# cvxopt/smcp

Hardware: AMD Instinct MI355X
Metric: Newton KKT solves/sec (higher is better)
Workload: dtype f64; 1 GPU; synth50k nested block-arrow SDP n=50000, 8073 cliques, m=100; kktsolver=chol, n=50000, cliques=8073, m=100, blkval_doubles=2493568, update_doubles=10689536, parallelism=single

## Files before the change

smcp_amd/csrc/capi.hip:

```cpp
#include <hip/hip_runtime.h>
#include <memory>
#include <unordered_map>

#include <algorithm>
#include <chrono>
#include <cstdio>
#include <cstring>
#include <map>
#include <new>
#include <atomic>
#include <thread>
#include <type_traits>
#include <vector>

#include "../../include/smcp_amd.h"
#include "context.hpp"
#include "switches.hpp"
#include "front_generic.hip"
#include "front_mfma.hip"
#include "front_large.hip"
#include "front_inv.hip"
#include "front_n16.hip"
#include "front_fam.hip"
#include "front_fam2.hip"
// ... 21 lines not shown
  KID_chol_level = 0, KID_llt_level, KID_pinv_level, KID_gather_level, KID_completion_all,
  KID_hess_up_level, KID_hess_down_level, KID_hess_down_inv_all, KID_hess_up_inv_level, KID_scale_an,
  KID_factor_yaa, KID_trsm_fwd_level, KID_trsm_bwd_level, KID_amap, KID_aadj, KID_scatter_constraints,
  KID_dense_potrf, KID_dense_potrs, KID_vec_axpby, KID_axpby, KID_reduce_cliques, KID_reduce_final,
  KID_hess_up_mfma, KID_hess_down_mfma, KID_chol_mfma, KID_pinv_mfma, KID_prep_lk,
  KID_hess_up_mfma_hbm, KID_hess_down_mfma_hbm, KID_chol_mfma_hbm, KID_pinv_mfma_hbm,
  KID_gram_partial, KID_gram_reduce, KID_hess_up_pad,
  KID_lf_assemble, KID_lf_clear_upd, KID_lf_up1, KID_lf_up2, KID_lf_up3, KID_lf_down1, KID_lf_down2, KID_lf_down3,
  KID_lf_pinv1, KID_lf_pinv2, KID_lf_diag, KID_lf_chol_panel, KID_lf_chol_trail, KID_lf_pack_upd,
  KID_lf_prep_s, KID_lf_prep_row, KID_lf_prep_k, KID_factor_yaa_lds,
  KID_factor_inverse, KID_hess_down_inv_mfma, KID_hess_down_inv_mfma_hbm, KID_hess_up_inv_mfma, KID_hess_up_inv_mfma_hbm,
  KID_completion_mfma, KID_completion_mfma_hbm, KID_lf_copy_an, KID_lf_ri_an, KID_lf_dinv1, KID_lf_dinv2,
  KID_lf_uinv1, KID_lf_uinv2, KID_lf_completion, KID_hess_up_n16, KID_llt_mfma, KID_llt_mfma_hbm, KID_lf_llt,
  KID_hess_up_fam, KID_qr_rmul, KID_qr_dots, KID_qr_comb, KID_qr_small, KID_fam2_prep, KID_mid_chol, KID_lf_diag_inv, KID_lfsp_up, KID_lfsp_prep, KID_leaf_gram, KID_leaf_tables, KID_fam_sparse, KID_gram_diag128, KID_lf_assemble_lds, KID_fam_terms, KID_famt_prep, KID_lf_assemble_lds_dyn, KID_lf_zsp, KID_fam_terms_grp, KID_lf_assemble_fz, KID_factor_inverse_lds, KID_chol_flow,
  KID_mrc_diag, KID_mrc_rank, KID_mrc_reduce, KID_mrc_factor, KID_cut_signs, KID_cut_weights,
  KID_edm_rank, KID_edm_reduce, KID_edm_factor, KID_edm_dense,
  KID_COUNT
};
const char* const KID_NAMES[KID_COUNT] = {
  "k_chol_level", "k_llt_level", "k_pinv_level", "k_gather_level", "k_completion_all",
  "k_hess_up_level", "k_hess_down_level", "k_hess_down_inv_all", "k_hess_up_inv_level", "k_scale_an",
  "k_factor_yaa", "k_trsm_fwd_level", "k_trsm_bwd_level", "k_amap", "k_aadj", "k_scatter_constraints",
  "k_dense_potrf", "k_dense_potrs", "k_vec_axpby", "k_axpby", "k_reduce_cliques", "k_reduce_final",
  "k_hess_up_mfma<true>", "k_hess_down_mfma<true>", "k_chol_mfma<true>", "k_pinv_mfma<true>", "k_prep_lk",
  "k_hess_up_mfma<false>", "k_hess_down_mfma<false>", "k_chol_mfma<false>", "k_pinv_mfma<false>",
  "k_gram_partial", "k_gram_reduce", "k_hess_up_pad",
  "k_lf_assemble", "k_lf_clear_upd", "k_lf_up1", "k_lf_up2", "k_lf_up3", "k_lf_down1", "k_lf_down2", "k_lf_down3",
  "k_lf_pinv1", "k_lf_pinv2", "k_lf_diag", "k_lf_chol_panel", "k_lf_chol_trail", "k_lf_pack_upd",
  "k_lf_prep_s", "k_lf_prep_row", "k_lf_prep_k", "k_factor_yaa_lds",
  "k_factor_inverse", "k_hess_down_inv_mfma<true>", "k_hess_down_inv_mfma<false>", "k_hess_up_inv_mfma<true>",
  "k_hess_up_inv_mfma<false>", "k_completion_mfma<true>", "k_completion_mfma<false>", "k_lf_copy_an", "k_lf_ri_an",
  "k_lf_dinv1", "k_lf_dinv2", "k_lf_uinv1", "k_lf_uinv2", "k_lf_completion", "k_hess_up_n16",
  "k_llt_mfma<true>", "k_llt_mfma<false>", "k_lf_llt", "k_hess_up_fam",
  "k_stack_trsm", "k_stack_dots", "k_stack_comb", "k_qr_small", "k_fam2_prep", "k_mid_chol", "k_lf_diag_inv", "k_lfsp_up", "k_lfsp_prep", "k_leaf_pairs", "k_leaf_tables", "k_fam_sparse", "k_gram_diag128", "k_lf_assemble_lds", "k_fam_terms", "k_famt_prep", "k_lf_assemble_lds_dyn", "k_lf_zsp", "k_fam_terms_grp", "k_lf_assemble_fz", "k_factor_inverse_lds", "k_chol_flow",
  "k_mrc_diag", "k_mrc_rank", "k_mrc_reduce", "k_mrc_factor", "k_cut_signs", "k_cut_weights",
  "k_edm_rank", "k_edm_reduce", "k_edm_factor", "k_edm_dense"};

inline void note_launch(csp_ctx* c, int kid) {
  const hipError_t e = hipGetLastError();
  if (e != hipSuccess && !c->launch_err) {
    c->launch_err = (int)e;
    fprintf(stderr, "smcp_amd: launch of %s failed: %s\n", (kid >= 0 && kid < KID_COUNT) ? KID_NAMES[kid] : "?", hipGetErrorString(e));
  }
}
inline hipError_t end_call(csp_ctx* c) {
  hipError_t e = hipGetLastError();
  if (e == hipSuccess && c->launch_err) e = c->launch_err > 0 ? (hipError_t)c->launch_err : hipErrorLaunchFailure;
  c->launch_err = 0;
  return e;
}

// ... 888 lines not shown
  DeviceCtx& D = c->D;
  const int cnn = std::max(1, a.famcnn), csa = 16 * std::max(1, (a.famcna + 15) / 16);
  const int64_t lim = (160 * 1024 - 1024) / 8;
  const int64_t fixed = fam2_layout<NAT>(cnn, csa).oTab;
  if (fixed + fam2_tail_doubles(4, 9) + 64 > lim) return false;
  static bool attr = false;
  if (!attr) {
    if (hipFuncSetAttribute((const void*)k_fam_sparse<NAT, KSN, true>, hipFuncAttributeMaxDynamicSharedMemorySize, 160 * 1024 - 1024) != hipSuccess) return false;
    if (hipFuncSetAttribute((const void*)k_fam_sparse<NAT, KSN, false>, hipFuncAttributeMaxDynamicSharedMemorySize, 160 * 1024 - 1024) != hipSuccess) return false;
    if (hipFuncSetAttribute((const void*)k_fam2_prep, hipFuncAttributeMaxDynamicSharedMemorySize, 160 * 1024 - 1024) != hipSuccess) return false;
    attr = true;
  }
  const int64_t need = (int64_t)cnt * fam2_const_doubles(cnn, csa);
  if (D.famc_len < need) {
    if (D.famc) { if (hipFree(D.famc) != hipSuccess) return false; D.bytes -= D.famc_len * 8; }
    D.famc = nullptr; D.famc_len = 0;
    if (dev_alloc(&D.famc, need, D.bytes)) return false;
    D.famc_len = need;
  }
  const int ncu = D.ncu;
  int g = 1;
  int64_t best = -1;
  for (int gc = 1; gc <= std::min(nrhs, 32); ++gc) {
    const int64_t rounds = ((int64_t)cnt * gc + ncu - 1) / ncu;
    const int64_t passes = (nrhs + gc - 1) / gc;
    const int64_t cost = rounds * ((passes + 1) / 2 + 4);
    if (best < 0 || cost < best) { best = cost; g = gc; }
  }
  const int passes = (nrhs + g - 1) / g;
  const double avg = 9.0 * (double)D.cnnz / ((double)c->S.nsn * (double)std::max<int64_t>(1, D.m));
  int tabpasses = std::min(passes, 113);
  while (tabpasses > 4 && fixed + fam2_tail_doubles(tabpasses, 9) + (int64_t)(1.5 * avg * tabpasses) + 8 > lim) tabpasses = (tabpasses + 1) / 2;
  const int64_t left = lim - fixed - fam2_tail_doubles(tabpasses, 9) - 4;
  const int ecap = (int)std::max<int64_t>(0, (left * 2) / 3 - 2);
  if (9 * D.kc_maxlist > ecap) return false;
  launch_lds(c, KID_fam2_prep, k_fam2_prep, dim3(cnt), dim3(512), (size_t)8 * fam2_child_layout(cnn, csa).cstride * sizeof(double), st,
             a, D.famc, cnn, csa);
  MfmaArgs a2 = a;
  { static int stag = -1; if (stag < 0) { const char* e = sw_str("SMCP_FAM2_STAG"); stag = e ? atoi(e) : 0; } a2.dn = stag; }
  if (D.lg_request) {
    launch_lds(c, KID_fam_sparse, k_fam_sparse<NAT, KSN, false>, dim3(cnt, g), dim3(512), (size_t)lim * 8, st, a2, U, ldu,
               (const double*)D.famc, cnn, csa, (const int32_t*)D.kc_ij, tabpasses, ecap);
    D.lg_nochild = true;
  } else {
    launch_lds(c, KID_fam_sparse, k_fam_sparse<NAT, KSN, true>, dim3(cnt, g), dim3(512), (size_t)lim * 8, st, a2, U, ldu,
               (const double*)D.famc, cnn, csa, (const int32_t*)D.kc_ij, tabpasses, ecap);
  }
  return true;
}
inline bool famt_disabled() {
// ... 10 lines not shown
  const int64_t lim = (160 * 1024 - 1024) / 8;
  const int64_t fixed = famt_layout<NAT>(8 * cnn).total + 8 * famt_desc_doubles() + famt_grp_misc_doubles();
  const int64_t left = lim - fixed - 4;
  if (left <= 0 || famt_prep_doubles<NAT>(cnn) > lim) return -1;
  return (int)std::max<int64_t>(0, (left * 2) / 3 - 2);
}
inline bool famt_grp_fits(int nat, int cnn) {
  int ecap = -1;
  switch (nat) {
    case 1: ecap = famt_grp_ecap<1>(cnn); break;
    case 2: ecap = famt_grp_ecap<2>(cnn); break;
    case 3: ecap = famt_grp_ecap<3>(cnn); break;
    case 4: ecap = famt_grp_ecap<4>(cnn); break;
  }
  return ecap >= FAMT_GMAX * (FAMT_TCAP / 2);
}
template <int NAT>
bool launch_famt(csp_ctx* c, const MfmaArgs& a, int cnt, int nrhs, double* U, int64_t ldu, hipStream_t st) {
  DeviceCtx& D = c->D;
  if (a.famt_ngrp > 0) {
    const int cnn = std::max(1, a.famcnn);
    const FamtL L = famt_layout<NAT>(8 * cnn);
    const int ecap = famt_grp_ecap<NAT>(cnn);
    static bool attrg = false;
    bool ok = !famt_disabled() && D.lg_request && D.fam_maxterms <= FAMT_TCAP / 2 && ecap >= FAMT_GMAX * (FAMT_TCAP / 2);
    if (ok && !attrg) {
      ok = hipFuncSetAttribute((const void*)k_fam_terms_grp<NAT>, hipFuncAttributeMaxDynamicSharedMemorySize, 160 * 1024 - 1024) == hipSuccess &&
           hipFuncSetAttribute((const void*)k_famt_prep<NAT>, hipFuncAttributeMaxDynamicSharedMemorySize, 160 * 1024 - 1024) == hipSuccess;
      attrg = ok;
    }
    const int64_t need = (int64_t)cnt * (FAMT_HDR + L.total);
    if (ok && D.famc_len < need) {
      if (D.famc) { if (hipFree(D.famc) != hipSuccess) ok = false; D.bytes -= D.famc_len * 8; }
      D.famc = nullptr; D.famc_len = 0;
      if (ok && dev_alloc(&D.famc, need, D.bytes)) ok = false;
      if (ok) D.famc_len = need;
    }
    if (!ok) {
      fprintf(stderr, "smcp_amd: grouped family sweep not launchable\n");
      if (!c->launch_err) c->launch_err = -1;
      return true;
    }
    const int gy = std::min(65535, (nrhs + 7) / 8);
    launch_lds(c, KID_famt_prep, k_famt_prep<NAT>, dim3(cnt), dim3(512), (size_t)famt_prep_doubles<NAT>(cnn) * sizeof(double), st, a, D.famc, cnn, (int32_t*)nullptr);
    launch_lds(c, KID_fam_terms_grp, k_fam_terms_grp<NAT>, dim3(a.famt_ngrp, gy), dim3(512), (size_t)(160 * 1024 - 1024), st, a, U, ldu,
               (const double*)D.famc, cnn, (const int32_t*)D.kc_ij, ecap);
    D.lg_nochild = true;
    return true;
  }
  if (famt_disabled() || !D.lg_request) return false;
  const int cnn = std::max(1, a.famcnn);
  const FamtL L = famt_layout<NAT>(8 * cnn);
  const int64_t lim = (160 * 1024 - 1024) / 8;
  const int64_t fixed = L.total + FAMT_NW * famt_desc_doubles() + 6;
  if (!famt_terms_ok(D)) return false;
  if (fixed + 9 * 4 + 64 > lim) return false;
  const int64_t prep_doubles = famt_prep_doubles<NAT>(cnn);
  if (prep_doubles > lim) return false;
  static bool attr = false;
  if (!attr) {
    if (hipFuncSetAttribute((const void*)k_fam_terms<NAT>, hipFuncAttributeMaxDynamicSharedMemorySize, 160 * 1024 - 1024) != hipSuccess) return false;
    if (hipFuncSetAttribute((const void*)k_famt_prep<NAT>, hipFuncAttributeMaxDynamicSharedMemorySize, 160 * 1024 - 1024) != hipSuccess) return false;
    attr = true;
  }
  const int64_t need = (int64_t)cnt * (FAMT_HDR + L.total);
  if (D.famc_len < need) {
    if (D.famc) { if (hipFree(D.famc) != hipSuccess) return false; D.bytes -= D.famc_len * 8; }
    D.famc = nullptr; D.famc_len = 0;
    if (dev_alloc(&D.famc, need, D.bytes)) return false;
    D.famc_len = need;
  }
  const int ncu = D.ncu;
  int g = 1;
  int64_t best = -1;
  for (int gc = 1; gc <= std::min(nrhs, 32); ++gc) {
    const int64_t rounds = ((int64_t)cnt * gc + ncu - 1) / ncu;
    const int64_t passes = (nrhs + gc - 1) / gc;
    const int64_t cost = rounds * (2 * ((passes + FAMT_NW - 1) / FAMT_NW) + 1);
    if (best < 0 || cost < best) { best = cost; g = gc; }
  }
  static int genv = -1;
  if (genv < 0) { const char* e = sw_str("SMCP_FAMT_G"); genv = e ? atoi(e) : 0; }
  if (genv > 0) g = std::min(genv, nrhs);
  const int passes = (nrhs + g - 1) / g;
  const double avg = 9.0 * (double)D.cnnz / ((double)c->S.nsn * (double)std::max<int64_t>(1, D.m));
  int tabpasses = std::min(passes, 113);
  auto tail = [&](int tp) { return (int64_t)2 * ((tp * 9 + 1) & ~1) / 2 + 2; };
  while (tabpasses > 4 && fixed + tail(tabpasses) + (int64_t)(1.5 * 1.5 * avg * tabpasses) + 8 > lim) tabpasses = (tabpasses + 1) / 2;
  const int64_t left = lim - fixed - tail(tabpasses) - 4;
  const int ecap = (int)std::max<int64_t>(0, (left * 2) / 3 - 2);
  if (9 * D.kc_maxlist > ecap) return false;
  if (a.fz_on) {
    static bool attrz = false;
    if (!attrz) attrz = hipFuncSetAttribute((const void*)k_fam_terms<NAT, false>, hipFuncAttributeMaxDynamicSharedMemorySize, 160 * 1024 - 1024) == hipSuccess;
    if (attrz && D.fz_slot) {
      launch_lds(c, KID_famt_prep, k_famt_prep<NAT>, dim3(cnt), dim3(512), (size_t)prep_doubles * sizeof(double), st, a, D.famc, cnn, D.fz_slot);
      launch_lds(c, KID_fam_terms, k_fam_terms<NAT, false>, dim3(cnt, g), dim3(64 * FAMT_NW), (size_t)lim * 8, st, a, U, ldu,
                 (const double*)D.famc, cnn, (const int32_t*)D.kc_ij, tabpasses, ecap);
      D.lg_nochild = true;
      c->fz_live = true; c->fz_nat = NAT; c->fz_cnn = cnn; c->fz_recl = (int64_t)(FAMT_HDR + L.total);
      return true;
    }
  }
  launch_lds(c, KID_famt_prep, k_famt_prep<NAT>, dim3(cnt), dim3(512), (size_t)prep_doubles * sizeof(double), st, a, D.famc, cnn, (int32_t*)nullptr);
  launch_lds(c, KID_fam_terms, k_fam_terms<NAT>, dim3(cnt, g), dim3(64 * FAMT_NW), (size_t)lim * 8, st, a, U, ldu,
             (const double*)D.famc, cnn, (const int32_t*)D.kc_ij, tabpasses, ecap);
  D.lg_nochild = true;
  return true;
}
inline bool fam2_disabled() {
  static int off = -1;
  if (off < 0) { const char* e = sw_str("SMCP_FAM2"); off = (e && e[0] == '0') ? 1 : 0; }
  return off != 0;
}
bool try_fam2(csp_ctx* c, const MfmaArgs& a, int cnt, int nrhs, double* U, int64_t ldu, hipStream_t st) {
  if (fam2_disabled() || !a.kc_ptr || !c->D.kc_ij || a.ymode != 2 || !a.ysc) return false;
  if (c->D.cnnz > (int64_t)4 * c->S.nsn * std::max<int64_t>(1, c->D.m)) return false;
  const int nat = std::max(1, (a.famna + 15) / 16);
  const bool k2 = a.famnn <= 8;
// ... 1263 lines not shown
      c->D.part_valid = false;
      fp_record(c, 2, x, st);
    }
    if (whole) fp_record(c, 1, x, st);
  } else
  for_levels_down(c, [&](const int32_t* lev, int cnt) {
    a.lev = lev;
    launch(c, KID_pinv_level, k_pinv_level, dim3(cnt), dim3(NT), st, a, x);
  });
  HIPCHK(end_call(c));
  return 0;
}

constexpr int SCALING_FAC = 1;
static bool leafgram_ok(csp_ctx* c, int64_t mcols);
static bool scaling_overlap_on() {
  static int on = -1;
  if (on < 0) { const char* e = sw_str("SMCP_SCALING_OVERLAP"); on = (e && e[0] == '0') ? 0 : 1; }
  return on == 1;
}
static int scaling_impl(csp_ctx* c, double* L, double* Y, int flags, hipStream_t st) {
  DeviceCtx& D = c->D;
  const Symbolic& S = c->S;
  const int64_t bl = S.blklen();
  if (c->scal_lstar < 0) {
    int64_t ls = S.nlev;
    while (ls > 0 && c->lvl[(size_t)ls - 1].nI == 0) --ls;
    c->scal_lstar = ls;
    std::vector<int> lev_of((size_t)S.nsn, 0);
    for (int64_t l = 0; l < S.nlev; ++l)
// ... 64 lines not shown
  bool skipped = false;
  auto factor_level = [&](int64_t l, hipStream_t lds_stream, hipStream_t large_stream) {
    for_level_classes(c, l, af, [&](bool lds, MfmaArgs am, int cnt, size_t, int) {
      if (!am.namax) return;
      if (lds) {
        if (l == 0 && skip_children && am.nS > 0) { cnt -= am.nS; skipped = true; if (!cnt) return; }
        const size_t bytes = ((size_t)padld(am.namax) * am.namax + 256 + 8) * sizeof(double);
        launch_lds(c, KID_factor_yaa_lds, k_factor_yaa_lds, dim3(cnt), dim3(fact_threads(am, 256, 2)), bytes, lds_stream, am, (const double*)D.yaa, D.fac);
      } else {
        launch(c, KID_axpby, k_copy_upd_blocks, dim3(cnt, umax1(std::min(64, (am.namax * am.namax + 1023) / 1024))), dim3(256), large_stream,
               am.t, (const double*)D.yaa, D.fac);
        lf_factor_yaa(c, am, cnt, D.fac, large_stream);
      }
    });
  };
  auto pinv_level = [&](int64_t l) {
    for_level_classes(c, l, ap, [&](bool lds, MfmaArgs am, int cnt, size_t bytes, int thr) {
      (void)bytes;
      if (lds) launch_lds(c, KID_pinv_mfma, k_pinv_mfma<true>, dim3(cnt), dim3(fact_threads(am, thr, 1)),
                          (size_t)mfma_lds_doubles_for(WK_PINV, am.nnmax, am.namax) * sizeof(double), st, am, Y);
      else lf_pinv(c, am, cnt, Y, st);
    });
  };
  for (int64_t l = last; l >= lstar; --l) pinv_level(l);
  bool any_large_sep = false;
  for (int64_t l = lstar; l <= last; ++l) if (c->lvl[(size_t)l].nII && c->lvl[(size_t)l].namaxII > 0) any_large_sep = true;
  std::unique_ptr<Fork> f1;
  if (want_fac && any_large_sep && lstar > 0) f1.reset(new Fork(c, st, 0));
  hipStream_t s1 = f1 ? f1->s : st;
  for (int64_t l = lstar - 1; l >= 0; --l) pinv_level(l);
  if (want_fac) {
    for (int64_t l = last; l >= lstar; --l) factor_level(l, s1, s1);
    for (int64_t l = lstar - 1; l >= 0; --l) factor_level(l, st, st);
  }
  if (f1) f1->join();
  D.lk_tag_L = L; D.lk_tag_Y = Y;
  D.yaa_tag = Y;
  D.fac_tag = want_fac ? Y : nullptr;
  D.fac_partial = want_fac && skipped;
  D.faci_tag = nullptr;
  if (want_fac) D.fac_gen++;
  HIPCHK(end_call(c));
  const int rc = fetch_info(c, st);
  if (rc) {
    D.lk_tag_L = D.lk_tag_Y = D.yaa_tag = D.fac_tag = D.faci_tag = nullptr;
    D.part_valid = false;
  }
  return rc;
}
int csp_cholesky_projected_inverse(csp_ctx* c, double* L, double* Y, int with_factors, void* stream) {
  if (int rc = ready(c)) return rc;
  if (!L || !Y || L == Y) return SMCP_EINVAL;
  return scaling_impl(c, L, Y, with_factors ? SCALING_FAC : 0, (hipStream_t)stream);
}

int csp_completion(csp_ctx* c, double* x, void* stream) {
  if (int rc = ready(c)) return rc;
  invalidate_tags(c, x);
  hipStream_t st = (hipStream_t)stream;
  TreeArgs a = tree_args(c);
// ... 654 lines not shown
```

smcp_amd/csrc/context.hpp:

```cpp
#pragma once
#include <hip/hip_runtime.h>

#include <cstdint>
#include <functional>
#include <map>
#include <vector>

#include "symbolic.hpp"

namespace smcp {

struct CliqueDesc {
  int64_t blk;
  int64_t upd;
  int64_t updp;
  int64_t rows;
  int64_t rel;
  int32_t nn, na;
  int32_t parent;
  int32_t chbeg, chend;
  int32_t first;
  int32_t pad;
};

// ... 51 lines not shown
  int32_t* a_c = nullptr;
  int32_t* s_rloc = nullptr;
  int32_t* s_cloc = nullptr;
  int32_t* dlist = nullptr;
  int32_t* slist = nullptr;
  int32_t* kidx = nullptr;
  int64_t md = 0, ns = 0;
  int32_t* kc_ptr = nullptr;
  int32_t* kc_off = nullptr;
  double* kc_val = nullptr;
  int32_t* kc_ij = nullptr;
  int32_t* fz_no = nullptr; int32_t* fz_slot = nullptr; int32_t* fz_ptr = nullptr; int32_t* fz_pk = nullptr; double* fz_s = nullptr;
  int64_t fz_nfam = 0; bool fz_ok = false;
  double* famc = nullptr;
  int64_t famc_len = 0;
  int64_t kc_maxlist = 0;
  int64_t fam_maxterms = 0;
  double fam_meanterms = 0;
  double* vbuf = nullptr;
  double* trsm_x = nullptr; int64_t trsm_x_len = 0;
  int64_t vcols = 0;
  double* hd = nullptr;
  double* hinv = nullptr;
  int64_t hinv_cap = 0, hinv_n = 0;
  const void* hinv_tag = nullptr;
  double* h_pending = nullptr; int64_t h_pending_n = 0, h_pending_ld = 0; hipStream_t h_pending_stream = nullptr;
  double* sw = nullptr;
  double* gpart = nullptr;
  int64_t gpart_len = 0;
  int64_t* gsl_start = nullptr; int32_t* gsl_len = nullptr; int64_t gsl_cap = 0; int gsl_n = 0;
// ... 124 lines not shown
```

smcp_amd/csrc/front_famt.hip:

```cpp
#include <hip/hip_runtime.h>

namespace smcp {

struct FamtL { int oLi, onK, onMK, oRt, oZero, oCN, oCA, oCM, total; };
template <int NAT>
__host__ __device__ inline FamtL famt_layout(int ncol) {
  constexpr int NA = 16 * NAT;
  FamtL L{};
  int o = 0;
  L.oLi = o; o += 256;
  L.onK = o; o += NA * 16;
  L.onMK = o; o += NA * 16;
  L.oRt = o; o += NA * NA;
  L.oZero = o; o += NA;
  L.oCN = o; o += ncol * 16;
  L.oCA = o; o += ncol * NA;
  L.oCM = o; o += ncol * NA;
  L.total = o;
  return L;
}
typedef unsigned int famt_u2 __attribute__((ext_vector_type(2)));
__device__ inline __amdgpu_buffer_rsrc_t famt_rsrc(double* base, int doubles) {
  return __builtin_amdgcn_make_buffer_rsrc(base, 0, doubles * 8, 0x00020000);
}
// ... 117 lines not shown
    hdr[0] = -1; hdr[1] = 1; hdr[2] = 0; hdr[3] = 0; hdr[4] = 0; hdr[5] = 0;
  }
  {
    const int used = __shfl(inc, 7);
    for (int e = tid; e < (ncol - used) * 16; e += 512) T[L.oCN + used * 16 + e] = 0.0;
    for (int e = tid; e < (ncol - used) * NA; e += 512) { T[L.oCA + used * NA + e] = 0.0; T[L.oCM + used * NA + e] = 0.0; }
  }
  if (tid == 0) {
    if (fz_slot && a.fz_no && a.fz_no[k] >= 0) fz_slot[a.fz_no[k]] = (int32_t)blockIdx.x;
    int* const hdr = reinterpret_cast<int*>(out);
    hdr[0] = k; hdr[1] = nn; hdr[2] = na; hdr[3] = nch;
    hdr[4] = (int)(d.blk & 0xffffffffll); hdr[5] = (int)(d.blk >> 32);
    hdr[6] = 0; hdr[7] = 0;
    hdr[8] = (int)(d.updp & 0xffffffffll); hdr[9] = (int)(d.updp >> 32);
  }
}

template <int NTH>
__device__ inline void famt_copy_tables(double* smem, const double* src, int total, int tid) {
  const double2* const s2 = reinterpret_cast<const double2*>(src);
  double2* const d2 = reinterpret_cast<double2*>(smem);
  const int n2 = total >> 1;
  for (int e0 = tid; e0 < n2; e0 += NTH * 8) {
    double2 v[8];
#pragma unroll
    for (int x = 0; x < 8; ++x) v[x] = s2[min(e0 + x * NTH, n2 - 1)];
#pragma unroll
    for (int x = 0; x < 8; ++x) if (e0 + x * NTH < n2) d2[e0 + x * NTH] = v[x];
  }
}
// ... 623 lines not shown
```

smcp_amd/csrc/kkt.hip:

```cpp

namespace {

using namespace smcp;

__global__ void __launch_bounds__(1024) k_amap(int64_t m, const int64_t* cptr, const int64_t* cidx, const double* cwval,
                                               const double* X, int64_t ldx, double* y, int64_t ldy, int64_t pstride) {
  __shared__ double part[16];
  const int lane = threadIdx.x & 63, wave = threadIdx.x >> 6, nthr = blockDim.x;
  const int64_t i = blockIdx.x;
  const int r = blockIdx.y;
  const double* x = X + (int64_t)r * ldx;
  const int64_t c0 = cptr[i], c1 = cptr[i + 1], share = (c1 - c0 + gridDim.z - 1) / gridDim.z;
  const int64_t e0 = c0 + (int64_t)blockIdx.z * share, e1 = e0 + share < c1 ? e0 + share : c1;
  y += (int64_t)blockIdx.z * pstride;
  double acc = 0.0;
  for (int64_t e = e0 + threadIdx.x; e < e1; e += 4 * nthr) {
    double w[4], v[4];
#pragma unroll
    for (int q = 0; q < 4; ++q) {
      const int64_t ee = e + (int64_t)q * nthr;
      w[q] = ee < e1 ? cwval[ee] : 0.0;
      v[q] = ee < e1 ? x[cidx[ee]] : 0.0;
    }
#pragma unroll
// ... 352 lines not shown
  if (m < 1 || !cptr || !cidx || !cval) return SMCP_EINVAL;
  DeviceCtx& D = c->D;
  const Symbolic& S = c->S;
  HIPCHK(hipSetDevice(D.device));
  if (D.h_pending) { if (int rc = flush_pending_potrf(c, D.h_pending_stream, nullptr, false)) return rc; }
  void* old[] = {D.fz_no, D.fz_slot, D.fz_ptr, D.fz_pk, D.fz_s, D.lg_eptr, D.lg_epk, D.lg_ew, D.lg_remap, D.lg_tab, D.cptr, D.cidx, D.cval, D.cwval, D.rpos, D.rptr, D.rcon, D.rval, D.ustack,
                 D.a_r, D.a_c, D.s_rloc, D.s_cloc, D.dlist, D.slist, D.kidx, D.vbuf, D.hd, D.kc_ptr, D.kc_off, D.kc_val, D.kc_ij, D.scm_owner};
  for (void* p : old) if (p) hipFree(p);
  D.cptr = nullptr; D.cidx = nullptr; D.cval = nullptr; D.cwval = nullptr; D.rpos = nullptr;
  D.rptr = nullptr; D.rcon = nullptr; D.rval = nullptr; D.ustack = nullptr;
  D.a_r = D.a_c = D.s_rloc = D.s_cloc = D.dlist = D.slist = D.kidx = nullptr;
  D.scm_owner = nullptr;
  D.vbuf = D.hd = nullptr;
  D.kc_ptr = D.kc_off = nullptr; D.kc_val = nullptr; D.kc_ij = nullptr;
  D.fz_no = D.fz_slot = D.fz_ptr = D.fz_pk = nullptr; D.fz_s = nullptr; D.fz_nfam = 0; D.fz_ok = false;
  D.md = D.ns = D.vcols = 0;
  D.lg_children = 0; D.lg_nochild = false;
  D.lg_eptr = D.lg_epk = D.lg_remap = nullptr; D.lg_ew = D.lg_tab = nullptr;
  c->gsl_key.clear();
  if (D.qr_ws) { hipFree(D.qr_ws); D.bytes -= D.qr_len * 8; D.qr_ws = nullptr; D.qr_len = 0; }
  D.qr_valid = false;
  SetupClock clk("kkt_set_constraints");
  const int64_t nnz = cptr[m];
  std::vector<double> w(nnz);
  std::vector<int32_t> ar(nnz), ac(nnz);
  std::vector<int32_t> ek(nnz), eoff(nnz);
  {
    const unsigned hw = std::thread::hardware_concurrency();
    const int nth = (int)std::max<int64_t>(1, std::min<int64_t>({(int64_t)(hw ? hw : 1), (int64_t)16, nnz / 65536 + 1}));
    std::atomic<int> bad{0};
// ... 1229 lines not shown
```

smcp_amd/csrc/switches.hpp:

```cpp
#pragma once
#include <cstdio>
#include <cstdlib>
#include <cstring>
#include <string>

extern char** environ;

namespace smcp {

struct Switch { const char* name; const char* dflt; const char* doc; };

static const Switch SWITCHES[] = {
  {"SMCP_GENERIC", "0", "1: any-size fixed-order kernels of front_generic.hip for every tree operation (as CSP_TUNE_DETERMINISTIC)"},
  {"SMCP_LARGE", "1", "0: no tiled large-front kernels (fronts beyond LDS take the one-workgroup HBM kernels)"},
  {"SMCP_NOCACHE", "0", "1: nothing derived from (L, Y) is reused between calls"},
  {"SMCP_FORK", "1", "0: no side streams, everything on the caller's stream"},
  {"SMCP_AUX_PRIO", "1", "0: side stream 0 (few-workgroup chains) at default instead of highest priority"},
  {"SMCP_AUX_PRIO1", "1", "0: side stream 1 (filler work) at default instead of lowest priority"},
  {"SMCP_EVENT_SYSFENCE", "0", "1: internal events with the default system-scope release (12 us per hand-over instead of 7)"},
  {"SMCP_SCALING_OVERLAP", "1", "0: csp_cholesky_projected_inverse as its three steps one after the other"},
  {"SMCP_CHOL_PREP", "1", "0: k_prep_lk in a launch of its own instead of inside k_chol_mfma (narrow supernodes)"},
  {"SMCP_FAC_PARTIAL", "1", "0: chol(Y_AA) of the family children always formed by the fused scaling point"},
  {"SMCP_MID", "1", "0: per-step kernels instead of k_mid_chol / k_lf_diag_inv for fronts of at most 272 rows"},
  {"SMCP_TRTRI", "1", "0: block-row triangular inversion of large fronts instead of recursive doubling"},
  {"SMCP_N16", "1", "0: no shape-specialised k_hess_up_n16"},
  {"SMCP_OLDLDS", "0", "1: k_hess_up_mfma<true> instead of the padded / n16 kernels"},
  {"SMCP_DOWN_W", "1", "0: k_hess_down_mfma instead of the one-wave k_hess_down_w"},
  {"SMCP_FAM", "1", "0: no family kernels (per-level sweeps with the update exchange through HBM)"},
  {"SMCP_FAM2", "1", "0: no sparse-input family kernels (k_fam_sparse, k_fam_terms): k_hess_up_fam"},
  {"SMCP_FAMT", "1", "0: no entry-driven family sweep k_fam_terms (k_fam_sparse instead)"},
  {"SMCP_FZ", "1", "0: the family parents' packed updates go through HBM (k_fam_terms writes, the extend-add reads) instead of being formed by k_lf_assemble_fz"},
  {"SMCP_FAMT_GROUP", "1", "0: no sibling groups of family parents (k_fam_terms_grp)"},
  {"SMCP_LFSP", "1", "0: dense phases instead of the sparse-input sweep k_lfsp_up of childless large fronts"},
  {"SMCP_LFSP_GROUP", "1", "0: no sibling groups in k_lfsp_up"},
  {"SMCP_ZSP", "1", "0: dense first phase of wide childless fronts instead of k_lf_zsp"},
  {"SMCP_LEAFGRAM", "1", "0: never the closed-form Gram blocks of the family children (k_leaf_tables / k_leaf_pairs)"},
  {"SMCP_LG_SIDE", "1", "0: leaf Gram blocks after the sweep on the caller's stream instead of beside the top phases"},
  {"SMCP_GRAM_EARLY", "0", "1: the Gram chunks of the levels 0 / 1 rows on the side branch beside the top fronts' phase kernels (measured slower: 3.37 against 3.22 ms per step)"},
  {"SMCP_LG_EARLY", "1", "0: leaf Gram blocks beside the phase kernels of the top fronts instead of from the start of the sweep"},
  {"SMCP_FACI_LDS", "1", "0: inverse Y_AA factors of the small fronts by block rows against HBM (k_factor_inverse) instead of in LDS"},
  {"SMCP_FZ_TAIL", "1", "0: every (front, right-hand side) pair of the fused extend-add is one workgroup's task, also in a thin last round"},
  {"SMCP_GRAM", "1", "0: reference (two-sweep) formulation of the Schur complement instead of the Gram formulation"},
  {"SMCP_SCM", "1", "0: column-sparse constraints swept like the others (no SCMcolumn2 route)"},
  {"SMCP_TRSM_MM", "1", "0: csp_trsm through the generic level kernels instead of tile products"},
  {"SMCP_ALDS", "1", "0: extend-add of large fronts by gather plan only (no LDS streaming kernel)"},
  {"SMCP_ALDS_DYN", "1", "0: one workgroup per (front, right-hand side) instead of the task-drawing grid"},
// ... 77 lines not shown
```

Measured before the change: 321.1 KKT solves/s.

## Form family records inside chol(Y_AA) of family parents and cache them for Schur call

Adds k_factor_yaa_famt, which factors Y_AA of the family-parent level and also writes the k_famt_prep records into the famc buffer during csp_cholesky_projected_inverse. A tag keyed on level, generations and pointers lets the later Schur-complement call skip the k_famt_prep launch when the records are still valid. The remaining levels' pinv and factor work is moved onto a forked stream so it runs beside the family level. This removes a separate prep kernel from the Schur path and overlaps lower-level work, at the cost of cache-invalidation complexity and a risk of stale records.

After: 328.6 KKT solves/s (median of 6 runs). +2.4%, better.

```diff
diff --git a/smcp_amd/csrc/capi.hip b/smcp_amd/csrc/capi.hip
--- a/smcp_amd/csrc/capi.hip
+++ b/smcp_amd/csrc/capi.hip
@@ -59,7 +59,7 @@
   KID_lf_uinv1, KID_lf_uinv2, KID_lf_completion, KID_hess_up_n16, KID_llt_mfma, KID_llt_mfma_hbm, KID_lf_llt,
   KID_hess_up_fam, KID_qr_rmul, KID_qr_dots, KID_qr_comb, KID_qr_small, KID_fam2_prep, KID_mid_chol, KID_lf_diag_inv, KID_lfsp_up, KID_lfsp_prep, KID_leaf_gram, KID_leaf_tables, KID_fam_sparse, KID_gram_diag128, KID_lf_assemble_lds, KID_fam_terms, KID_famt_prep, KID_lf_assemble_lds_dyn, KID_lf_zsp, KID_fam_terms_grp, KID_lf_assemble_fz, KID_factor_inverse_lds, KID_chol_flow,
   KID_mrc_diag, KID_mrc_rank, KID_mrc_reduce, KID_mrc_factor, KID_cut_signs, KID_cut_weights,
-  KID_edm_rank, KID_edm_reduce, KID_edm_factor, KID_edm_dense,
+  KID_edm_rank, KID_edm_reduce, KID_edm_factor, KID_edm_dense, KID_factor_yaa_famt,
   KID_COUNT
 };
 const char* const KID_NAMES[KID_COUNT] = {
@@ -79,7 +79,7 @@
   "k_llt_mfma<true>", "k_llt_mfma<false>", "k_lf_llt", "k_hess_up_fam",
   "k_stack_trsm", "k_stack_dots", "k_stack_comb", "k_qr_small", "k_fam2_prep", "k_mid_chol", "k_lf_diag_inv", "k_lfsp_up", "k_lfsp_prep", "k_leaf_pairs", "k_leaf_tables", "k_fam_sparse", "k_gram_diag128", "k_lf_assemble_lds", "k_fam_terms", "k_famt_prep", "k_lf_assemble_lds_dyn", "k_lf_zsp", "k_fam_terms_grp", "k_lf_assemble_fz", "k_factor_inverse_lds", "k_chol_flow",
   "k_mrc_diag", "k_mrc_rank", "k_mrc_reduce", "k_mrc_factor", "k_cut_signs", "k_cut_weights",
-  "k_edm_rank", "k_edm_reduce", "k_edm_factor", "k_edm_dense"};
+  "k_edm_rank", "k_edm_reduce", "k_edm_factor", "k_edm_dense", "k_factor_yaa_famt"};
 
 inline void note_launch(csp_ctx* c, int kid) {
   const hipError_t e = hipGetLastError();
@@ -998,7 +998,7 @@
   const int64_t need = (int64_t)cnt * fam2_const_doubles(cnn, csa);
   if (D.famc_len < need) {
     if (D.famc) { if (hipFree(D.famc) != hipSuccess) return false; D.bytes -= D.famc_len * 8; }
-    D.famc = nullptr; D.famc_len = 0;
+    D.famc = nullptr; D.famc_len = 0; D.famc_tag = DeviceCtx::FamcTag();
     if (dev_alloc(&D.famc, need, D.bytes)) return false;
     D.famc_len = need;
   }
@@ -1018,6 +1018,7 @@
   const int64_t left = lim - fixed - fam2_tail_doubles(tabpasses, 9) - 4;
   const int ecap = (int)std::max<int64_t>(0, (left * 2) / 3 - 2);
   if (9 * D.kc_maxlist > ecap) return false;
+  D.famc_tag = DeviceCtx::FamcTag();
   launch_lds(c, KID_fam2_prep, k_fam2_prep, dim3(cnt), dim3(512), (size_t)8 * fam2_child_layout(cnn, csa).cstride * sizeof(double), st,
              a, D.famc, cnn, csa);
   MfmaArgs a2 = a;
@@ -1058,6 +1059,33 @@
     case 4: ecap = famt_grp_ecap<4>(cnn); break;
   }
   return ecap >= FAMT_GMAX * (FAMT_TCAP / 2);
+}
+inline int famt_layout_total(int nat, int cnn) {
+  switch (nat) {
+    case 1: return famt_layout<1>(8 * cnn).total;
+    case 2: return famt_layout<2>(8 * cnn).total;
+    case 3: return famt_layout<3>(8 * cnn).total;
+    case 4: return famt_layout<4>(8 * cnn).total;
+  }
+  return 0;
+}
+inline bool famt_early_on() {
+  static int on = -1;
+  if (on < 0) on = sw_on("SMCP_FAMT_EARLY", 1);
+  return on == 1;
+}
+inline bool famc_cached(const csp_ctx* c, const MfmaArgs& a, int cnt, int nat, int cnn) {
+  const DeviceCtx& D = c->D;
+  const DeviceCtx::FamcTag& t = D.famc_tag;
+  return famt_early_on() && !cache_off() && t.lev && t.lev == a.t.lev && t.cnt == cnt && t.nat == nat && t.cnn == cnn &&
+         t.lk_gen == D.lk_gen && t.fac_gen == D.fac_gen && t.cset_gen == D.cset_gen && t.L == D.lk_tag_L && t.Y == D.fac_tag &&
+         a.ysc == D.fac && !D.part_valid && D.famc_len >= (int64_t)cnt * (FAMT_HDR + famt_layout_total(nat, cnn));
+}
+template <int NAT>
+void famt_records(csp_ctx* c, const MfmaArgs& a, int cnt, int cnn, int32_t* fz_slot, hipStream_t st) {
+  if (famc_cached(c, a, cnt, NAT, cnn)) return;
+  c->D.famc_tag = DeviceCtx::FamcTag();
+  launch_lds(c, KID_famt_prep, k_famt_prep<NAT>, dim3(cnt), dim3(512), (size_t)famt_prep_doubles<NAT>(cnn) * sizeof(double), st, a, c->D.famc, cnn, fz_slot);
 }
 template <int NAT>
 bool launch_famt(csp_ctx* c, const MfmaArgs& a, int cnt, int nrhs, double* U, int64_t ldu, hipStream_t st) {
@@ -1076,7 +1104,7 @@
     const int64_t need = (int64_t)cnt * (FAMT_HDR + L.total);
     if (ok && D.famc_len < need) {
       if (D.famc) { if (hipFree(D.famc) != hipSuccess) ok = false; D.bytes -= D.famc_len * 8; }
-      D.famc = nullptr; D.famc_len = 0;
+      D.famc = nullptr; D.famc_len = 0; D.famc_tag = DeviceCtx::FamcTag();
       if (ok && dev_alloc(&D.famc, need, D.bytes)) ok = false;
       if (ok) D.famc_len = need;
     }
@@ -1086,7 +1114,7 @@
       return true;
     }
     const int gy = std::min(65535, (nrhs + 7) / 8);
-    launch_lds(c, KID_famt_prep, k_famt_prep<NAT>, dim3(cnt), dim3(512), (size_t)famt_prep_doubles<NAT>(cnn) * sizeof(double), st, a, D.famc, cnn, (int32_t*)nullptr);
+    famt_records<NAT>(c, a, cnt, cnn, (int32_t*)nullptr, st);
     launch_lds(c, KID_fam_terms_grp, k_fam_terms_grp<NAT>, dim3(a.famt_ngrp, gy), dim3(512), (size_t)(160 * 1024 - 1024), st, a, U, ldu,
                (const double*)D.famc, cnn, (const int32_t*)D.kc_ij, ecap);
     D.lg_nochild = true;
@@ -1110,7 +1138,7 @@
   const int64_t need = (int64_t)cnt * (FAMT_HDR + L.total);
   if (D.famc_len < need) {
     if (D.famc) { if (hipFree(D.famc) != hipSuccess) return false; D.bytes -= D.famc_len * 8; }
-    D.famc = nullptr; D.famc_len = 0;
+    D.famc = nullptr; D.famc_len = 0; D.famc_tag = DeviceCtx::FamcTag();
     if (dev_alloc(&D.famc, need, D.bytes)) return false;
     D.famc_len = need;
   }
@@ -1138,7 +1166,7 @@
     static bool attrz = false;
     if (!attrz) attrz = hipFuncSetAttribute((const void*)k_fam_terms<NAT, false>, hipFuncAttributeMaxDynamicSharedMemorySize, 160 * 1024 - 1024) == hipSuccess;
     if (attrz && D.fz_slot) {
-      launch_lds(c, KID_famt_prep, k_famt_prep<NAT>, dim3(cnt), dim3(512), (size_t)prep_doubles * sizeof(double), st, a, D.famc, cnn, D.fz_slot);
+      famt_records<NAT>(c, a, cnt, cnn, D.fz_slot, st);
       launch_lds(c, KID_fam_terms, k_fam_terms<NAT, false>, dim3(cnt, g), dim3(64 * FAMT_NW), (size_t)lim * 8, st, a, U, ldu,
                  (const double*)D.famc, cnn, (const int32_t*)D.kc_ij, tabpasses, ecap);
       D.lg_nochild = true;
@@ -1146,7 +1174,7 @@
       return true;
     }
   }
-  launch_lds(c, KID_famt_prep, k_famt_prep<NAT>, dim3(cnt), dim3(512), (size_t)prep_doubles * sizeof(double), st, a, D.famc, cnn, (int32_t*)nullptr);
+  famt_records<NAT>(c, a, cnt, cnn, (int32_t*)nullptr, st);
   launch_lds(c, KID_fam_terms, k_fam_terms<NAT>, dim3(cnt, g), dim3(64 * FAMT_NW), (size_t)lim * 8, st, a, U, ldu,
              (const double*)D.famc, cnn, (const int32_t*)D.kc_ij, tabpasses, ecap);
   D.lg_nochild = true;
@@ -2440,6 +2468,25 @@
 
 constexpr int SCALING_FAC = 1;
 static bool leafgram_ok(csp_ctx* c, int64_t mcols);
+static int64_t famt_early_lds(int nat, int cnn) {
+  switch (nat) {
+    case 1: return famt_early_doubles<1>(cnn);
+    case 2: return famt_early_doubles<2>(cnn);
+    case 3: return famt_early_doubles<3>(cnn);
+    case 4: return famt_early_doubles<4>(cnn);
+  }
+  return INT64_MAX;
+}
+static bool famt_early_attr(int nat) {
+  static int ok[5] = {-1, -1, -1, -1, -1};
+  if (nat < 1 || nat > 4) return false;
+  if (ok[nat] < 0) {
+    const void* f = nat == 1 ? (const void*)k_factor_yaa_famt<1> : nat == 2 ? (const void*)k_factor_yaa_famt<2> :
+                    nat == 3 ? (const void*)k_factor_yaa_famt<3> : (const void*)k_factor_yaa_famt<4>;
+    ok[nat] = hipFuncSetAttribute(f, hipFuncAttributeMaxDynamicSharedMemorySize, 160 * 1024 - 1024) == hipSuccess ? 1 : 0;
+  }
+  return ok[nat] == 1;
+}
 static bool scaling_overlap_on() {
   static int on = -1;
   if (on < 0) { const char* e = sw_str("SMCP_SCALING_OVERLAP"); on = (e && e[0] == '0') ? 0 : 1; }
@@ -2534,24 +2581,87 @@
       }
     });
   };
-  auto pinv_level = [&](int64_t l) {
+  auto pinv_level = [&](int64_t l, hipStream_t s) {
     for_level_classes(c, l, ap, [&](bool lds, MfmaArgs am, int cnt, size_t bytes, int thr) {
       (void)bytes;
       if (lds) launch_lds(c, KID_pinv_mfma, k_pinv_mfma<true>, dim3(cnt), dim3(fact_threads(am, thr, 1)),
-                          (size_t)mfma_lds_doubles_for(WK_PINV, am.nnmax, am.namax) * sizeof(double), st, am, Y);
-      else lf_pinv(c, am, cnt, Y, st);
+                          (size_t)mfma_lds_doubles_for(WK_PINV, am.nnmax, am.namax) * sizeof(double), s, am, Y);
+      else lf_pinv(c, am, cnt, Y, s);
     });
   };
-  for (int64_t l = last; l >= lstar; --l) pinv_level(l);
+  D.famc_tag = DeviceCtx::FamcTag();
+  int64_t famlev = -1;
+  int famnat = 0, famcnn = 0;
+  if (want_fac && famt_early_on() && D.m > 0 && !D.ns && D.kc_ptr && D.kc_ij && leafgram_ok(c, D.m) && !famt_disabled() && !fam2_disabled() &&
+      famt_terms_ok(D) && D.cnnz <= (int64_t)4 * S.nsn * std::max<int64_t>(1, D.m)) {
+    int nfamlev = 0;
+    for (int64_t l = 1; l < lstar; ++l)
+      for_level_classes(c, l, af, [&](bool lds, MfmaArgs am, int, size_t, int) {
+        if (!lds || am.nS <= 0) return;
+        ++nfamlev; famlev = l;
+        famnat = std::max(1, (am.famna + 15) / 16); famcnn = std::max(1, am.famcnn);
+      });
+    const int64_t lim = (160 * 1024 - 1024) / 8;
+    if (nfamlev != 1 || famnat > 4 || famt_early_lds(famnat, famcnn) > lim || !famt_early_attr(famnat)) famlev = -1;
+  }
+  auto famt_factor = [&](MfmaArgs am, int cnt) {
+    const int nS = am.nS;
+    const int64_t need = (int64_t)nS * (FAMT_HDR + famt_layout_total(famnat, famcnn));
+    if (D.famc_len < need) {
+      if (D.famc) { if (hipFree(D.famc) != hipSuccess) return false; D.bytes -= D.famc_len * 8; }
+      D.famc = nullptr; D.famc_len = 0;
+      if (dev_alloc(&D.famc, need, D.bytes)) return false;
+      D.famc_len = need;
+    }
+    am.t.lev = am.t.lev + (cnt - nS);
+    const size_t bytes = (size_t)famt_early_lds(famnat, famcnn) * sizeof(double);
+    switch (famnat) {
+      case 1: launch_lds(c, KID_factor_yaa_famt, k_factor_yaa_famt<1>, dim3(nS), dim3(256), bytes, st, am, (const double*)D.yaa, D.fac, D.famc, famcnn, (const int32_t*)D.fz_no, D.fz_slot); break;
+      case 2: launch_lds(c, KID_factor_yaa_famt, k_factor_yaa_famt<2>, dim3(nS), dim3(256), bytes, st, am, (const double*)D.yaa, D.fac, D.famc, famcnn, (const int32_t*)D.fz_no, D.fz_slot); break;
+      case 3: launch_lds(c, KID_factor_yaa_famt, k_factor_yaa_famt<3>, dim3(nS), dim3(256), bytes, st, am, (const double*)D.yaa, D.fac, D.famc, famcnn, (const int32_t*)D.fz_no, D.fz_slot); break;
+      case 4: launch_lds(c, KID_factor_yaa_famt, k_factor_yaa_famt<4>, dim3(nS), dim3(256), bytes, st, am, (const double*)D.yaa, D.fac, D.famc, famcnn, (const int32_t*)D.fz_no, D.fz_slot); break;
+    }
+    D.famc_tag.lev = am.t.lev; D.famc_tag.cnt = nS; D.famc_tag.nat = famnat; D.famc_tag.cnn = famcnn;
+    return true;
+  };
+  for (int64_t l = last; l >= lstar; --l) pinv_level(l, st);
   bool any_large_sep = false;
   for (int64_t l = lstar; l <= last; ++l) if (c->lvl[(size_t)l].nII && c->lvl[(size_t)l].namaxII > 0) any_large_sep = true;
   std::unique_ptr<Fork> f1;
   if (want_fac && any_large_sep && lstar > 0) f1.reset(new Fork(c, st, 0));
   hipStream_t s1 = f1 ? f1->s : st;
-  for (int64_t l = lstar - 1; l >= 0; --l) pinv_level(l);
-  if (want_fac) {
+  if (famlev < 0) {
+    for (int64_t l = lstar - 1; l >= 0; --l) pinv_level(l, st);
+    if (want_fac) {
+      for (int64_t l = last; l >= lstar; --l) factor_level(l, s1, s1);
+      for (int64_t l = lstar - 1; l >= 0; --l) factor_level(l, st, st);
+    }
+  } else {
+    for (int64_t l = lstar - 1; l >= famlev; --l) pinv_level(l, st);
+    Fork fe(c, st, 1);
+    for (int64_t l = lstar - 1; l > famlev; --l) factor_level(l, st, st);
+    for_level_classes(c, famlev, af, [&](bool lds, MfmaArgs am, int cnt, size_t, int) {
+      if (!am.namax) return;
+      if (lds && am.nS > 0) {
+        int rest = cnt;
+        if (famt_factor(am, cnt)) rest -= am.nS;
+        if (rest > 0) {
+          const size_t bytes = ((size_t)padld(am.namax) * am.namax + 256 + 8) * sizeof(double);
+          launch_lds(c, KID_factor_yaa_lds, k_factor_yaa_lds, dim3(rest), dim3(fact_threads(am, 256, 2)), bytes, st, am, (const double*)D.yaa, D.fac);
+        }
+      } else if (lds) {
+        const size_t bytes = ((size_t)padld(am.namax) * am.namax + 256 + 8) * sizeof(double);
+        launch_lds(c, KID_factor_yaa_lds, k_factor_yaa_lds, dim3(cnt), dim3(fact_threads(am, 256, 2)), bytes, st, am, (const double*)D.yaa, D.fac);
+      } else {
+        launch(c, KID_axpby, k_copy_upd_blocks, dim3(cnt, umax1(std::min(64, (am.namax * am.namax + 1023) / 1024))), dim3(256), st,
+               am.t, (const double*)D.yaa, D.fac);
+        lf_factor_yaa(c, am, cnt, D.fac, st);
+      }
+    });
     for (int64_t l = last; l >= lstar; --l) factor_level(l, s1, s1);
-    for (int64_t l = lstar - 1; l >= 0; --l) factor_level(l, st, st);
+    for (int64_t l = famlev - 1; l >= 0; --l) pinv_level(l, fe.s);
+    for (int64_t l = famlev - 1; l >= 0; --l) factor_level(l, fe.s, fe.s);
+    fe.join();
   }
   if (f1) f1->join();
   D.lk_tag_L = L; D.lk_tag_Y = Y;
@@ -2560,10 +2670,15 @@
   D.fac_partial = want_fac && skipped;
   D.faci_tag = nullptr;
   if (want_fac) D.fac_gen++;
+  if (D.famc_tag.lev) {
+    D.famc_tag.lk_gen = D.lk_gen; D.famc_tag.fac_gen = D.fac_gen; D.famc_tag.cset_gen = D.cset_gen;
+    D.famc_tag.L = L; D.famc_tag.Y = Y;
+  }
   HIPCHK(end_call(c));
   const int rc = fetch_info(c, st);
   if (rc) {
     D.lk_tag_L = D.lk_tag_Y = D.yaa_tag = D.fac_tag = D.faci_tag = nullptr;
+    D.famc_tag = DeviceCtx::FamcTag();
     D.part_valid = false;
   }
   return rc;
diff --git a/smcp_amd/csrc/context.hpp b/smcp_amd/csrc/context.hpp
--- a/smcp_amd/csrc/context.hpp
+++ b/smcp_amd/csrc/context.hpp
@@ -89,6 +89,9 @@
   int64_t fz_nfam = 0; bool fz_ok = false;
   double* famc = nullptr;
   int64_t famc_len = 0;
+  struct FamcTag { const int32_t* lev = nullptr; int cnt = 0, nat = 0, cnn = 0; int64_t lk_gen = -1, fac_gen = -1, cset_gen = -1; const void* L = nullptr; const void* Y = nullptr; };
+  FamcTag famc_tag;
+  int64_t cset_gen = 0;
   int64_t kc_maxlist = 0;
   int64_t fam_maxterms = 0;
   double fam_meanterms = 0;
diff --git a/smcp_amd/csrc/front_famt.hip b/smcp_amd/csrc/front_famt.hip
--- a/smcp_amd/csrc/front_famt.hip
+++ b/smcp_amd/csrc/front_famt.hip
@@ -155,6 +155,138 @@
     hdr[6] = 0; hdr[7] = 0;
     hdr[8] = (int)(d.updp & 0xffffffffll); hdr[9] = (int)(d.updp >> 32);
   }
+}
+
+template <int NAT>
+__host__ __device__ inline int famt_early_doubles(int cnn) {
+  constexpr int NA = 16 * NAT;
+  return padld(NA) * NA + 264 + 256 + NA * 16 + 8 * cnn * (16 + NA);
+}
+template <int NAT>
+__global__ void __launch_bounds__(256) k_factor_yaa_famt(MfmaArgs a, const double* yaa, double* fac, double* famt, int cnn,
+                                                         const int32_t* fz_no, int32_t* fz_slot) {
+  extern __shared__ __attribute__((aligned(16))) double smem[];
+  constexpr int NA = 16 * NAT, ld = NA | 1;
+  const int ncol = 8 * cnn;
+  const FamtL L = famt_layout<NAT>(ncol);
+  const int k = a.t.lev[blockIdx.x];
+  const CliqueDesc d = a.t.cl[k];
+  const int nn = d.nn, na = d.na, nf = nn + na, nch = d.chend - d.chbeg;
+  const int tid = threadIdx.x, lane = tid & 63, wave = tid >> 6, nth = blockDim.x;
+  double* const M = smem;
+  double* const D16 = M + ld * NA;
+  double* const sLi = D16 + 264;
+  double* const snK = sLi + 256;
+  double* const sQN = snK + NA * 16;
+  double* const sA = sQN + 16 * ncol;
+  double* const out = famt + (int64_t)blockIdx.x * (FAMT_HDR + L.total);
+  double* const T = out + FAMT_HDR;
+  const int myck = lane < nch ? a.t.chidx[d.chbeg + lane] : 0;
+  const int mynn = lane < nch ? a.t.cl[myck].nn : 0;
+  int inc = mynn;
+#pragma unroll
+  for (int o = 1; o < 8; o <<= 1) { const int v = __shfl_up(inc, o); if (lane >= o) inc += v; }
+  {
+    const double* src = yaa + d.upd;
+    batched_loop<8>(tid, na * na, nth, [=](int e) { return (e % na) >= (e / na) ? src[e] : 0.0; },
+                    [=](int e, double v) { M[(e % na) + (e / na) * ld] = v; });
+  }
+  for (int e = tid; e < 256 + NA * 16 + ncol * (16 + NA); e += nth) sLi[e] = 0.0;
+  if (wave == 0 && lane < 8) {
+    int* const hdr = reinterpret_cast<int*>(out) + 16 + 6 * lane;
+    if (lane < nch) { hdr[0] = myck; hdr[1] = mynn; hdr[2] = a.t.cl[myck].na; hdr[3] = inc - mynn; }
+    else { hdr[0] = -1; hdr[1] = 1; hdr[2] = 0; hdr[3] = 0; }
+    hdr[4] = 0; hdr[5] = 0;
+  }
+  if (tid == 0) {
+    if (fz_slot && fz_no && fz_no[k] >= 0) fz_slot[fz_no[k]] = (int32_t)blockIdx.x;
+    int* const hdr = reinterpret_cast<int*>(out);
+    hdr[0] = k; hdr[1] = nn; hdr[2] = na; hdr[3] = nch;
+    hdr[4] = (int)(d.blk & 0xffffffffll); hdr[5] = (int)(d.blk >> 32);
+    hdr[6] = 0; hdr[7] = 0;
+    hdr[8] = (int)(d.updp & 0xffffffffll); hdr[9] = (int)(d.updp >> 32);
+  }
+  __syncthreads();
+  {
+    const double* lk = a.LK + d.blk;
+    batched_loop<8>(tid, nf * nn, nth, [=](int e) { return lk[e]; },
+                    [=](int e, double v) {
+                      const int i = e % nf, j = e / nf;
+                      if (i >= nn) snK[(i - nn) + j * NA] = -v;
+                      else if (i >= j) sLi[i + j * 16] = v;
+                    });
+    for (int c = wave; c < nch; c += nth >> 6) {
+      const int ck = __shfl(myck, c), colbase = __shfl(inc - mynn, c);
+      const CliqueDesc cd = a.t.cl[ck];
+      const int nnc = cd.nn, nac = cd.na, nfc = nnc + nac;
+      if (lane < nac) {
+        const int rel = a.t.relidx[cd.rel + lane];
+        const double* lkc = a.LK + cd.blk + nnc + lane;
+        double* const dst = rel < nn ? sQN + rel + 16 * colbase : sA + (rel - nn) + NA * colbase;
+        const int ldd = rel < nn ? 16 : NA;
+        for (int j0 = 0; j0 < nnc; j0 += 8) {
+          double kv[8];
+#pragma unroll
+          for (int x = 0; x < 8; ++x) kv[x] = j0 + x < nnc ? lkc[(int64_t)(j0 + x) * nfc] : 0.0;
+#pragma unroll
+          for (int x = 0; x < 8; ++x) if (j0 + x < nnc) dst[ldd * (j0 + x)] = kv[x];
+        }
+      }
+    }
+  }
+  __syncthreads();
+  wg_mma(16 + NA, ncol, 16, [=](int m, int kk) { return m < 16 ? sLi[m + 16 * kk] : snK[(m - 16) + kk * NA]; },
+         [=](int kk, int g) { return sQN[kk + 16 * g]; },
+         [=](int m, int g, double acc) {
+           if (m < 16) T[L.oCN + g * 16 + m] = acc;
+           else {
+             const double v = sA[(m - 16) + NA * g] + acc;
+             sA[(m - 16) + NA * g] = v;
+             T[L.oCA + g * NA + (m - 16)] = v;
+           }
+         });
+  for (int jb = 0; jb < na; jb += 16) {
+    const int bw = min(16, na - jb);
+    int f = potrf_inv16(M + jb + jb * ld, ld, bw, D16);
+    if (f) { if (tid == 0) atomicCAS(info_of(a.t, k), 0, info_val(a.t, k)); return; }
+    const int mrem = na - jb - bw;
+    if (mrem > 0) {
+      double* Pj = M + (jb + bw) + jb * ld;
+      wg_mma(mrem, bw, bw, [=](int m, int kk) { return Pj[m + kk * ld]; },
+             [=](int kk, int n) { return D16[n + kk * 16]; },
+             [=](int m, int n, double acc) { Pj[m + n * ld] = acc; });
+      __syncthreads();
+      double* Tr = M + (jb + bw) + (jb + bw) * ld;
+      wg_mma(mrem, mrem, bw, [=](int m, int kk) { return Pj[m + kk * ld]; },
+             [=](int kk, int n) { return Pj[n + kk * ld]; },
+             [=](int m, int n, double acc) { if (m >= n) Tr[m + n * ld] -= acc; }, true);
+      __syncthreads();
+    }
+  }
+  __syncthreads();
+  {
+    double* dst = fac + d.upd;
+    for (int e = tid; e < na * na; e += nth) {
+      const int i = e % na, j = e / na;
+      if (i >= j) dst[e] = M[i + j * ld];
+    }
+  }
+  wg_mma(NA, 16 + ncol, na, [=](int p, int q) { return (p < na && q >= p) ? M[q + p * ld] : 0.0; },
+         [=](int q, int n) { return n < 16 ? snK[q + n * NA] : sA[q + NA * (n - 16)]; },
+         [=](int p, int n, double acc) {
+           if (n < 16) T[L.onMK + n * NA + p] = acc;
+           else T[L.oCM + (n - 16) * NA + p] = acc;
+         });
+  double2* const T2 = reinterpret_cast<double2*>(T);
+  for (int e = tid; e < 128; e += nth) T2[(L.oLi >> 1) + e] = make_double2(sLi[2 * e], sLi[2 * e + 1]);
+  for (int e = tid; e < NA * 8; e += nth) T2[(L.onK >> 1) + e] = make_double2(snK[2 * e], snK[2 * e + 1]);
+  for (int e = tid; e < NA * NA / 2; e += nth) {
+    const int p = (2 * e) % NA, q = (2 * e) / NA;
+    const double v0 = (q < na && q >= p) ? M[q + p * ld] : 0.0;
+    const double v1 = (q < na && q >= p + 1) ? M[q + (p + 1) * ld] : 0.0;
+    T2[(L.oRt >> 1) + e] = make_double2(v0, v1);
+  }
+  for (int e = tid; e < NA / 2; e += nth) T2[(L.oZero >> 1) + e] = make_double2(0.0, 0.0);
 }
 
 template <int NTH>
diff --git a/smcp_amd/csrc/kkt.hip b/smcp_amd/csrc/kkt.hip
--- a/smcp_amd/csrc/kkt.hip
+++ b/smcp_amd/csrc/kkt.hip
@@ -390,6 +390,8 @@
   D.vbuf = D.hd = nullptr;
   D.kc_ptr = D.kc_off = nullptr; D.kc_val = nullptr; D.kc_ij = nullptr;
   D.fz_no = D.fz_slot = D.fz_ptr = D.fz_pk = nullptr; D.fz_s = nullptr; D.fz_nfam = 0; D.fz_ok = false;
+  D.cset_gen++;
+  D.famc_tag = DeviceCtx::FamcTag();
   D.md = D.ns = D.vcols = 0;
   D.lg_children = 0; D.lg_nochild = false;
   D.lg_eptr = D.lg_epk = D.lg_remap = nullptr; D.lg_ew = D.lg_tab = nullptr;
diff --git a/smcp_amd/csrc/switches.hpp b/smcp_amd/csrc/switches.hpp
--- a/smcp_amd/csrc/switches.hpp
+++ b/smcp_amd/csrc/switches.hpp
@@ -30,6 +30,7 @@
   {"SMCP_FAM2", "1", "0: no sparse-input family kernels (k_fam_sparse, k_fam_terms): k_hess_up_fam"},
   {"SMCP_FAMT", "1", "0: no entry-driven family sweep k_fam_terms (k_fam_sparse instead)"},
   {"SMCP_FZ", "1", "0: the family parents' packed updates go through HBM (k_fam_terms writes, the extend-add reads) instead of being formed by k_lf_assemble_fz"},
+  {"SMCP_FAMT_EARLY", "1", "0: the family records (k_famt_prep) formed in the Schur call instead of with chol(Y_AA) of the family parents in csp_cholesky_projected_inverse (k_factor_yaa_famt)"},
   {"SMCP_FAMT_GROUP", "1", "0: no sibling groups of family parents (k_fam_terms_grp)"},
   {"SMCP_LFSP", "1", "0: dense phases instead of the sparse-input sweep k_lfsp_up of childless large fronts"},
   {"SMCP_LFSP_GROUP", "1", "0: no sibling groups in k_lfsp_up"},
```
